# keras-team/keras-rs

Measured on AMD Instinct MI355X. Metric: embedding lookups/sec + DCN fwd+bwd step time, 26-table DLRM batch 65 536, higher is better.
Workload: dtype bf16; 1 GPU; C3 DLRM-small: 26 tables x 1000000 rows x 128 (bf16), global batch 65536, multi-hot ml_perf lengths (sum L = 214), uniform ids, DotInteraction(F=27) + 3 x FeatureCross(d=3456, projection=512), fused Adagrad on tables; global_batch=65536, parallelism=single GPU

## Files before the change

include/krs.h:

```cpp
#ifndef KRS_H_
#define KRS_H_

#include <stddef.h>
#include <stdint.h>

#ifdef __cplusplus
extern "C" {
#endif

#define KRS_VERSION 100

typedef enum krs_status {
  KRS_OK = 0,
  KRS_ERR_INVALID = -1,
  KRS_ERR_UNSUPPORTED = -2,
  KRS_ERR_LAUNCH = -3,
  KRS_ERR_WORKSPACE = -4
} krs_status;

typedef enum krs_dtype { KRS_F32 = 0, KRS_BF16 = 1, KRS_I8 = 2 } krs_dtype;
typedef enum krs_itype { KRS_I32 = 0, KRS_I64 = 1 } krs_itype;

typedef enum krs_combiner { KRS_SUM = 0, KRS_MEAN = 1, KRS_SQRTN = 2 } krs_combiner;

// ... 169 lines not shown
int krs_gemm_dense_bwd(const void* a, int64_t lda, const void* bt, int64_t ldb, void* g_out, int64_t ldg,
                       const void* y, void* dz, int64_t ld, float* dbias, int64_t m, int64_t n, int64_t k, int act,
                       int dtype, void* workspace, size_t workspace_bytes, void* stream);
enum { KRS_CROSS_BWD_NONE = 0, KRS_CROSS_BWD_TWO_CALL = 1, KRS_CROSS_BWD_PP64 = 2, KRS_CROSS_BWD_PP256 = 3 };
int krs_gemm_cross_bwd_last_route(int* epilogue);
int krs_gemm_cross_bwd_plan_route(const void* a, int64_t lda, const void* bt, int64_t ldb, const void* r, int64_t ldr,
                                  float beta, void* g_out, int64_t ldg, const void* x0, const void* u, void* dz, void* dx0,
                                  int64_t ld, int dx0_accumulate, const void* u_upper, int64_t m, int64_t n, int64_t k,
                                  int dtype, int* epilogue);

enum {
  KRS_GEMM_KERNEL_NONE = 0, KRS_GEMM_KERNEL_GENERIC = 1, KRS_GEMM_KERNEL_MFMA = 2, KRS_GEMM_KERNEL_GLDS = 3,
  KRS_GEMM_KERNEL_TN_GLDS = 4, KRS_GEMM_KERNEL_PP256 = 5, KRS_GEMM_KERNEL_PP256_KSTRIDED = 6, KRS_GEMM_KERNEL_PP64 = 7,
  KRS_GEMM_KERNEL_THIN = 8, KRS_GEMM_KERNEL_ROWDOT = 9, KRS_GEMM_KERNEL_SMALLK = 10
};
enum { KRS_GEMM_REDUCE_NONE = 0, KRS_GEMM_REDUCE_SCALAR = 1, KRS_GEMM_REDUCE_VEC4 = 2, KRS_GEMM_REDUCE_VEC8 = 3 };
typedef struct krs_gemm_route {
  int32_t kernel;
  int32_t splits;
  int32_t reduce;
  int32_t epilogue;
  int32_t ep_vec;
  int32_t thin_width;
  int32_t thin_is_a;
} krs_gemm_route;
int krs_gemm_last_route(krs_gemm_route* route);
int krs_gemm_plan_route(const void* a, int64_t lda, int a_is_km, const void* b, int64_t ldb, int b_is_nk, const void* c,
                        int64_t ldc, int64_t m, int64_t n, int64_t k, int in_dtype, int out_dtype,
                        const krs_gemm_epilogue* epilogue, size_t workspace_bytes, krs_gemm_route* route);

enum { KRS_GEMM_OPT_PIPELINE = 0 };
int krs_gemm_set_option(int key, int value);

enum { KRS_EMBED_OPT_PLAN = 2, KRS_EMBED_OPT_HOTROWS = 3, KRS_EMBED_OPT_RANK = 4, KRS_EMBED_OPT_APPLY_DEPTH = 5 };
int krs_embed_set_option(int key, int value);

size_t krs_colsum_workspace_bytes(int64_t m, int64_t n);
int krs_cross_epilogue_fwd(const void* u, const void* x0, const void* x, void* y,
                           int64_t m, int64_t n, int64_t ld, float diag_scale,
                           int dtype, void* stream);
int krs_cross_epilogue_bwd(const void* g, const void* u, const void* x0, const void* x,
                           void* du, void* dx0, int dx0_accumulate, void* dxd,
                           float* dbias,
                           int64_t m, int64_t n, int64_t ld, float diag_scale, int act,
                           int dtype, void* workspace, size_t workspace_bytes, void* stream);

int krs_cast_transpose(const void* src, int64_t rows, int64_t cols, int64_t ld_src, int src_dtype,
                       void* dst, int64_t ld_dst, void* dst_t, int64_t ld_dst_t, int dst_dtype,
                       void* stream);
int krs_cast_transpose_many(int count, const void* const* srcs, const int64_t* rows, const int64_t* cols,
                            int src_dtype, void* const* dsts, void* const* dst_ts, int dst_dtype, void* stream);

int krs_dense_act_bwd(const void* g, int64_t ld_g, const void* y, int64_t ld_y, void* dz, int64_t ld_dz,
                      float* dbias, int64_t m, int64_t n, int act, int dtype, void* workspace,
                      size_t workspace_bytes, void* stream);

int krs_dense_adagrad(float* const* params, const float* const* grads, float* const* accs,
                      const int64_t* sizes, int count, float lr, float eps, void* stream);

int krs_colsum(const void* a, int64_t lda, int64_t m, int64_t n, int dtype,
               float* out, void* workspace, size_t workspace_bytes, void* stream);

int krs_dot_interaction_fwd(const void* const* feats, const int64_t* ld, int n_feats,
                            int64_t batch, int dim, int dtype,
                            int self_interaction, int skip_gather,
                            void* out, int64_t out_ld, void* stream);
int krs_dot_interaction_bwd(const void* const* feats, const int64_t* ld, int n_feats,
// ... 150 lines not shown
```

keras_rs_amd/csrc/embed_bag_fwd.hip:

```cpp
#include <cstdlib>

#include "embed_fwd_plan.h"
#include "krs_common.h"

namespace krs {
namespace {

typedef uint32_t u32x4 __attribute__((ext_vector_type(4)));
typedef float f32x4 __attribute__((ext_vector_type(4)));
constexpr int NT = 2;

struct EmbedFwdParams {
  const krs_table* tables;
  const krs_feature* feats;
  int n_feats;
  const void* ids;
  int id64;
  const void* offsets;
  int off64;
  const float* weights;
  int batch;
  int dim;
  void* out;
  int64_t out_ld;
// ... 521 lines not shown
    if constexpr (sizeof(TT) == 2 && sizeof(OT) == 2 && LPR == 16) {
      if (rt.hot_rows == 128) {
        if (rt.stream) hipLaunchKernelGGL((embed_bag_fwd_vec<TT, OT, LPR, false, true, 128>), grid, block, 0, st, p);
        else hipLaunchKernelGGL((embed_bag_fwd_vec<TT, OT, LPR, false, false, 128>), grid, block, 0, st, p);
      } else {
        if (rt.stream) hipLaunchKernelGGL((embed_bag_fwd_vec<TT, OT, LPR, false, true, 64>), grid, block, 0, st, p);
        else hipLaunchKernelGGL((embed_bag_fwd_vec<TT, OT, LPR, false, false, 64>), grid, block, 0, st, p);
      }
      KRS_CHECK_LAUNCH("embed_bag_fwd_vec (hot rows in LDS)");
      return KRS_OK;
    } else {
      return fail(KRS_ERR_UNSUPPORTED, "embed_bag_fwd: hot rows are staged for bf16 rows of 256 bytes only");
    }
  }
#define KRS_K1_LAUNCH(W, S) hipLaunchKernelGGL((embed_bag_fwd_vec<TT, OT, LPR, W, S>), grid, block, 0, st, p)
  if (rt.has_w) { if (rt.stream) KRS_K1_LAUNCH(true, true); else KRS_K1_LAUNCH(true, false); }
  else { if (rt.stream) KRS_K1_LAUNCH(false, true); else KRS_K1_LAUNCH(false, false); }
#undef KRS_K1_LAUNCH
  KRS_CHECK_LAUNCH("embed_bag_fwd_vec");
  return KRS_OK;
}

template <typename TT, typename OT>
int launch_vec(const EmbedFwdParams& p, const krs_embed_fwd_route& rt, hipStream_t st) {
  if (rt.lpr == 8) return launch_lpr<TT, OT, 8>(p, rt, st);
  if (rt.lpr == 16) return launch_lpr<TT, OT, 16>(p, rt, st);
  if (rt.lpr == 32) return launch_lpr<TT, OT, 32>(p, rt, st);
  return launch_lpr<TT, OT, 64>(p, rt, st);
}

}
}

namespace krs { extern int g_plan_variant, g_rank_mode; }
namespace krs { int g_apply_depth = 4; }

extern "C" int krs_embed_set_option(int key, int value) {
  if (key == KRS_EMBED_OPT_PLAN) {
    KRS_REQUIRE(value == 0 || value == 1, "krs_embed_set_option: plan variant must be 0 or 1");
    krs::g_plan_variant = value;
    return KRS_OK;
  }
  if (key == KRS_EMBED_OPT_RANK) {
    KRS_REQUIRE(value >= 0 && value <= 2, "krs_embed_set_option: rank mode must be 0, 1 or 2");
    krs::g_rank_mode = value;
    return KRS_OK;
  }
  if (key == KRS_EMBED_OPT_HOTROWS) {
    KRS_REQUIRE(value == 0 || value == 64 || value == 128, "krs_embed_set_option: hot rows must be 0, 64 or 128");
    krs::g_hot_rows = value;
    return KRS_OK;
  }
  if (key == KRS_EMBED_OPT_APPLY_DEPTH) {
    KRS_REQUIRE(value == 0 || value == 4 || value == 8 || value == 16,
                "krs_embed_set_option: apply depth must be 0, 4, 8 or 16");
    krs::g_apply_depth = value;
    return KRS_OK;
  }
  return krs::fail(KRS_ERR_INVALID, "krs_embed_set_option: unknown key %d", key);
}

extern "C" int krs_embed_bag_fwd(const krs_table* tables, const krs_feature* feats, int n_feats,
                                 const void* ids, int id_type, const void* offsets, int off_type,
                                 const float* weights, int64_t nnz, int batch, int dim,
                                 int table_dtype, void* out, int out_dtype, int64_t out_ld,
                                 float* bag_scale, int* err_flag, void* stream) {
  using namespace krs;
  g_route = krs_embed_fwd_route{};
  KRS_REQUIRE(tables && feats && out, "embed_bag_fwd: null tables/feats/out");
  KRS_REQUIRE(ids || nnz == 0, "embed_bag_fwd: null ids");
  eplan::EmbedFwdPlan pl;
  if (int rc = embed_fwd_plan(n_feats, offsets, weights, nnz, batch, dim, table_dtype, out, out_dtype, out_ld, pl)) return rc;
  KRS_REQUIRE((id_type == KRS_I32 || id_type == KRS_I64) && (off_type == KRS_I32 || off_type == KRS_I64),
              "embed_bag_fwd: bad index type");
  const krs_embed_fwd_route& rt = pl.route;
  if (rt.kernel == KRS_EMBED_FWD_NONE) return KRS_OK;
  hipStream_t st = reinterpret_cast<hipStream_t>(stream);

// ... 36 lines not shown
```

keras_rs_amd/csrc/embed_bag_plan.hip:

```cpp
#include <algorithm>

#include "krs_bag_plan.h"

namespace krs {
int g_plan_variant = 0;
int g_rank_mode = 0;
namespace {

namespace rs {
constexpr int kHistThreads = 256, kHistItems = kTile / kHistThreads;
constexpr int kThreads = 512, kWaves = kThreads / 64, kItems = kTile / kThreads;
constexpr int kGenFeats = 256;

struct Gen {
  const krs_table* tables;
  const krs_feature* feats;
  int n_feats;
  const void* ids;
  int id64;
  int batch;
  int* err_flag;
};

struct alignas(16) GenLds {
  uint32_t base[kGenFeats + 1];
  uint32_t hot[kGenFeats];
  uint32_t row_base[kGenFeats];
  uint32_t vocab[kGenFeats];
};
__device__ __forceinline__ void load_gen(const Gen& gen, int64_t nnz, GenLds& g, int n_threads) {
  for (int i = threadIdx.x; i <= gen.n_feats; i += n_threads) {
    if (i < gen.n_feats) {
      const krs_feature ft = gen.feats[i];
      const krs_table tb = gen.tables[ft.table];
      g.base[i] = (uint32_t)ft.ids_base;
      g.hot[i] = (uint32_t)ft.hot;
      g.row_base[i] = (uint32_t)tb.row_base;
      g.vocab[i] = (uint32_t)tb.vocab;
    } else {
      g.base[i] = (uint32_t)nnz;
    }
  }
}
__device__ __forceinline__ int gen_feature(const GenLds& g, int n_feats, uint32_t q) {
  int lo = 0, hi = n_feats;
  while (hi - lo > 1) {
    const int mid = (lo + hi) >> 1;
    if (g.base[mid] <= q) lo = mid; else hi = mid;
  }
  return lo;
}
__device__ __forceinline__ uint64_t gen_value(const Gen& gen, const GenLds& g, int f, uint32_t q) {
  const uint32_t bag = (uint32_t)f * (uint32_t)gen.batch + (q - g.base[f]) / g.hot[f];
  return ((uint64_t)bag << 32) | (uint64_t)q;
}
__device__ __forceinline__ bool generate(const Gen& gen, const GenLds& g, uint32_t q, uint32_t& key, uint64_t& val) {
  const int f = gen_feature(g, gen.n_feats, q);
  const int64_t id = ld_index(gen.ids, gen.id64, q);
  const bool valid = id >= 0 && id < (int64_t)g.vocab[f];
  key = valid ? g.row_base[f] + (uint32_t)id : kInvalidKey;
  val = gen_value(gen, g, f, q);
  return valid;
}

__device__ __forceinline__ int digit_of(uint32_t key, int shift, int bins) { return (int)((key >> shift) & (bins - 1)); }

__device__ __forceinline__ uint32_t tile_of_block(uint32_t b, uint32_t tiles) { return (b & 7) * ((tiles + 7) / 8) + (b >> 3); }
inline unsigned tile_grid(unsigned tiles) { return (tiles + 7) / 8 * 8; }

__device__ __forceinline__ void hist_zero(int (&h)[kMaxBins], int bins) {
  for (int i = threadIdx.x; i < bins; i += kHistThreads) h[i] = 0;
}
__device__ __forceinline__ void hist_add(int (&h)[kMaxBins], uint32_t key, int shift, int bins) {
  atomicAdd(&h[digit_of(key, shift, bins)], 1);
}
__device__ __forceinline__ void hist_finish(const int (&h)[kMaxBins], int bins, int32_t* col, int64_t stride, bool bad,
                                            int* err_flag) {
  if (bad && err_flag) atomicOr(err_flag, KRS_FLAG_ID_OUT_OF_RANGE);
  __syncthreads();
  for (int i = threadIdx.x; i < bins; i += kHistThreads) col[(int64_t)i * stride] = h[i];
}

template <typename V>
struct alignas(16) TileLds {
  uint16_t cnt[kWaves][kMaxBins];
  uint16_t tile_excl[kMaxBins];
  int gbase[kMaxBins];
  uint32_t skey[kTile];
  V sval[kTile];
  int wtot[kWaves];
};
template <typename V>
__device__ __forceinline__ void zero_counts(TileLds<V>& s) {
  for (int i = threadIdx.x; i < kWaves * kMaxBins; i += kThreads) (&s.cnt[0][0])[i] = 0;
}
// ... 110 lines not shown
    }
  }
  __syncthreads();
}
template <typename V>
__device__ __forceinline__ void stage_tile(TileLds<V>& s, const uint32_t (&key)[kItems], const V (&val)[kItems],
                                           const int (&rank)[kItems], int64_t first, int64_t end, int shift, int bins) {
  const int wave = threadIdx.x >> 6;
#pragma unroll
  for (int it = 0; it < kItems; ++it) {
    if (first + it * 64 < end) {
      const int lp = s.cnt[wave][digit_of(key[it], shift, bins)] + rank[it];
      s.skey[lp] = key[it];
      s.sval[lp] = val[it];
    }
  }
  __syncthreads();
}
template <typename V>
__device__ __forceinline__ int out_slot(const TileLds<V>& s, int i, int d) {
  return s.gbase[d] + (i - (int)s.tile_excl[d]);
}

struct Pass {
  const uint32_t* keys_in;
  const uint64_t* vals_in;
  uint32_t* keys_out;
  uint64_t* vals_out;
  int32_t* counts;
  int64_t nnz;
  int n_tiles;
  int shift, bits;
  int rank;
  Gen gen;
};

template <bool GEN>
__global__ __launch_bounds__(kHistThreads) void hist_kernel(const Pass p) {
  __shared__ int h[kMaxBins];
  __shared__ GenLds g;
  const uint32_t tile = tile_of_block(blockIdx.x, p.n_tiles);
  if (tile >= (uint32_t)p.n_tiles) return;
  const int bins = 1 << p.bits;
  hist_zero(h, bins);
  if constexpr (GEN) load_gen(p.gen, p.nnz, g, kHistThreads);
  __syncthreads();
  const int64_t base = (int64_t)tile * kTile;
  bool bad = false;
  for (int it = 0; it < kHistItems; ++it) {
    const int64_t q = base + it * kHistThreads + threadIdx.x;
    if (q < p.nnz) {
      uint32_t key;
      if constexpr (GEN) {
        uint64_t v;
        bad |= !generate(p.gen, g, (uint32_t)q, key, v);
      } else {
        key = p.keys_in[q];
      }
      hist_add(h, key, p.shift, bins);
    }
  }
  hist_finish(h, bins, p.counts + tile, p.n_tiles, bad, p.gen.err_flag);
}

template <bool GEN>
__global__ __launch_bounds__(kThreads) void scatter_kernel(const Pass p) {
  __shared__ TileLds<uint64_t> s;
  __shared__ GenLds g;
  const uint32_t tile = tile_of_block(blockIdx.x, p.n_tiles);
  if (tile >= (uint32_t)p.n_tiles) return;
  const int bins = 1 << p.bits;
  zero_counts(s);
  if constexpr (GEN) load_gen(p.gen, p.nnz, g, kThreads);
  __syncthreads();
  const int lane = threadIdx.x & 63, wave = threadIdx.x >> 6;
  const int64_t tile0 = (int64_t)tile * kTile;
  const int64_t first = tile0 + (int64_t)wave * (kTile / kWaves) + lane;
  uint32_t key[kItems];
  uint64_t val[kItems];
  int rank[kItems];
#pragma unroll
  for (int it = 0; it < kItems; ++it) {
    const int64_t q = first + it * 64;
    const bool live = q < p.nnz;
    key[it] = kInvalidKey;
    val[it] = 0;
    if (live) {
      if constexpr (GEN) {
        generate(p.gen, g, (uint32_t)q, key[it], val[it]);
      } else {
        key[it] = p.keys_in[q];
        val[it] = p.vals_in[q];
      }
    }
  }
  rank_keys(key, first, p.nnz, p.shift, p.bits, p.rank, s.cnt[wave], lane, rank);
  digit_bases(s, bins, p.counts + tile, p.n_tiles);
  stage_tile(s, key, val, rank, first, p.nnz, p.shift, bins);
  const int n_here = (int)min<int64_t>(kTile, p.nnz - tile0);
#pragma unroll
  for (int it = 0; it < kItems; ++it) {
    const int i = it * kThreads + threadIdx.x;
    if (i < n_here) {
      const uint32_t k = s.skey[i];
      const int pos = out_slot(s, i, digit_of(k, p.shift, bins));
      p.keys_out[pos] = k;
      p.vals_out[pos] = s.sval[i];
    }
  }
}

struct Seg {
  int n;
  uint32_t lookup_start[kMaxProb + 1];
  uint32_t tile_start[kMaxProb + 1];
  uint32_t row_base[kMaxProb];
};
struct SegPass {
  const uint32_t* keys_in;
  const uint32_t* pos_in;
  uint32_t* keys_out;
  uint32_t* pos_out;
  uint64_t* vals_out;
  int32_t* counts;
  int64_t nnz;
  int shift, bits, key_bits;
  int rank;
  Gen gen;
  Seg seg;
};
struct SegTile {
  int pr;
  int64_t t0, end;
  int32_t* col;
  uint32_t stride;
};
__device__ __forceinline__ SegTile seg_tile(const SegPass& p, uint32_t tile) {
  const Seg& sg = p.seg;
  int lo = 0, hi = sg.n;
  while (hi - lo > 1) {
    const int mid = (lo + hi) >> 1;
    if (sg.tile_start[mid] <= tile) lo = mid; else hi = mid;
  }
  SegTile t;
  t.pr = lo;
  const uint32_t tl = tile - sg.tile_start[lo];
  t.stride = sg.tile_start[lo + 1] - sg.tile_start[lo];
  t.t0 = (int64_t)sg.lookup_start[lo] + (int64_t)tl * kTile;
  t.end = min<int64_t>(t.t0 + kTile, sg.lookup_start[lo + 1]);
  t.col = p.counts + ((int64_t)1 << p.bits) * sg.tile_start[lo] + tl;
  return t;
}
template <int ITEMS, int STRIDE>
__device__ __forceinline__ bool seg_first_keys(const SegPass& p, const GenLds& g, const SegTile& t, int64_t first,
                                               uint32_t (&key)[ITEMS], uint32_t (&pos)[ITEMS]) {
  int64_t idv[ITEMS];
#pragma unroll
  for (int it = 0; it < ITEMS; ++it) idv[it] = ld_index(p.gen.ids, p.gen.id64, min<int64_t>(first + it * STRIDE, t.end - 1));
  const int f_lo = gen_feature(g, p.gen.n_feats, (uint32_t)t.t0), f_hi = gen_feature(g, p.gen.n_feats, (uint32_t)(t.end - 1));
  bool bad = false;
#pragma unroll
  for (int it = 0; it < ITEMS; ++it) {
    const int64_t q = min<int64_t>(first + it * STRIDE, t.end - 1);
    const int f = f_lo == f_hi ? f_lo : gen_feature(g, p.gen.n_feats, (uint32_t)q);
    const bool valid = idv[it] >= 0 && idv[it] < (int64_t)g.vocab[f];
    key[it] = valid ? (uint32_t)idv[it] : (1u << p.key_bits) - 1u;
    pos[it] = (uint32_t)q;
    bad = bad || (!valid && first + it * STRIDE < t.end);
  }
  return bad;
}

template <bool FIRST>
__global__ __launch_bounds__(kHistThreads) void hist_seg_kernel(const SegPass p) {
  __shared__ int h[kMaxBins];
  __shared__ GenLds g;
  const uint32_t tile = tile_of_block(blockIdx.x, p.seg.tile_start[p.seg.n]);
  if (tile >= p.seg.tile_start[p.seg.n]) return;
  const int bins = 1 << p.bits;
  hist_zero(h, bins);
  if constexpr (FIRST) load_gen(p.gen, p.nnz, g, kHistThreads);
  __syncthreads();
  const SegTile t = seg_tile(p, tile);
  const int64_t first = t.t0 + threadIdx.x;
  bool bad = false;
  uint32_t key[kHistItems];
  if constexpr (FIRST) {
    uint32_t pos[kHistItems];
    bad = seg_first_keys<kHistItems, kHistThreads>(p, g, t, first, key, pos);
  } else {
#pragma unroll
    for (int it = 0; it < kHistItems; ++it) key[it] = p.keys_in[min<int64_t>(first + it * kHistThreads, t.end - 1)];
  }
#pragma unroll
  for (int it = 0; it < kHistItems; ++it)
    if (first + it * kHistThreads < t.end) hist_add(h, key[it], p.shift, bins);
  hist_finish(h, bins, t.col, t.stride, bad, p.gen.err_flag);
}

template <bool FIRST, bool LAST>
__global__ __launch_bounds__(kThreads) void scatter_seg_kernel(const SegPass p) {
  __shared__ TileLds<uint32_t> s;
  __shared__ GenLds g;
  const uint32_t tile = tile_of_block(blockIdx.x, p.seg.tile_start[p.seg.n]);
  if (tile >= p.seg.tile_start[p.seg.n]) return;
  const int bins = 1 << p.bits;
  zero_counts(s);
  if constexpr (FIRST || LAST) load_gen(p.gen, p.nnz, g, kThreads);
  __syncthreads();
  const int lane = threadIdx.x & 63, wave = threadIdx.x >> 6;
  const SegTile t = seg_tile(p, tile);
  const int64_t first = t.t0 + (int64_t)wave * (kTile / kWaves) + lane;
  uint32_t key[kItems], pos[kItems];
  int rank[kItems];
  if constexpr (FIRST) {
    seg_first_keys<kItems, 64>(p, g, t, first, key, pos);
  } else {
#pragma unroll
    for (int it = 0; it < kItems; ++it) {
      const int64_t q = min<int64_t>(first + it * 64, t.end - 1);
      key[it] = p.keys_in[q];
      pos[it] = p.pos_in[q];
    }
  }
#pragma unroll
  for (int it = 0; it < kItems; ++it) {
    const bool live = first + it * 64 < t.end;
    if (!live) { key[it] = 0xffffffffu; pos[it] = 0; }
  }
  rank_keys(key, first, t.end, p.shift, p.bits, p.rank, s.cnt[wave], lane, rank);
  digit_bases(s, bins, t.col, t.stride);
  stage_tile(s, key, pos, rank, first, t.end, p.shift, bins);
  const int n_here = (int)(t.end - t.t0);
  const uint32_t sentinel = (1u << p.key_bits) - 1u, rb = p.seg.row_base[t.pr];
  int pf_lo = 0, pf_hi = 1;
  if constexpr (LAST) {
    pf_lo = gen_feature(g, p.gen.n_feats, p.seg.lookup_start[t.pr]);
    pf_hi = gen_feature(g, p.gen.n_feats, p.seg.lookup_start[t.pr + 1] - 1);
  }
#pragma unroll
  for (int it = 0; it < kItems; ++it) {
    const int i = it * kThreads + threadIdx.x;
    if (i < n_here) {
      const uint32_t k = s.skey[i], q = s.sval[i];
      const int o = out_slot(s, i, digit_of(k, p.shift, bins));
      if constexpr (LAST) {
        const int f = pf_lo == pf_hi ? pf_lo : gen_feature(g, p.gen.n_feats, q);
        p.keys_out[o] = k == sentinel ? kInvalidKey : rb + k;
        p.vals_out[o] = gen_value(p.gen, g, f, q);
      } else {
        p.keys_out[o] = k;
        p.pos_out[o] = q;
      }
    }
  }
}

inline unsigned key_bits(int64_t n) {
  unsigned bits = 1;
  while (bits < 32 && (1ULL << bits) <= (uint64_t)n) ++bits;
  return bits;
}
struct Schedule {
  int passes;
  int bits[4], shift[4];
};
inline Schedule pass_schedule(unsigned bits) {
  Schedule s;
  s.passes = (int)((bits + kMaxBits - 1) / kMaxBits);
  unsigned done = 0;
  for (int ps = 0; ps < s.passes; ++ps) {
    s.bits[ps] = (int)((bits - done + (s.passes - ps) - 1) / (s.passes - ps));
    s.shift[ps] = (int)done;
    done += (unsigned)s.bits[ps];
  }
  return s;
}
inline Gen make_gen(const krs_table* tables, const krs_feature* feats, int n_feats, const void* ids, int id_type,
                    int batch, int* err_flag) {
  Gen g;
  g.tables = tables; g.feats = feats; g.n_feats = n_feats; g.ids = ids;
  g.id64 = id_type == KRS_I64; g.batch = batch; g.err_flag = err_flag;
  return g;
}
}

struct KeyParams {
  const krs_table* tables;
  const krs_feature* feats;
  int n_feats;
  const void* ids;
  int id64;
  const void* offsets;
  int off64;
  int batch;
  uint32_t* keys;
  uint64_t* vals;
  int* err_flag;
};

__global__ __launch_bounds__(256) void bag_keys_kernel(const KeyParams p) {
  const int64_t bag = (int64_t)blockIdx.x * 16 + (threadIdx.x >> 4);
  const int sub = threadIdx.x & 15;
  if (bag >= (int64_t)p.n_feats * p.batch) return;
  const int f = (int)(bag / p.batch);
  const int b = (int)(bag - (int64_t)f * p.batch);
  const krs_feature ft = p.feats[f];
  const krs_table tb = p.tables[ft.table];
  int64_t s, e;
  if (p.offsets) {
    s = ld_index(p.offsets, p.off64, bag);
    e = ld_index(p.offsets, p.off64, bag + 1);
  } else {
    s = ft.ids_base + (int64_t)b * ft.hot;
    e = s + ft.hot;
// ... 57 lines not shown
#pragma unroll
  for (int o = 1; o < 64; o <<= 1) {
    const int y = __shfl_up(x, o, 64);
    if (lane >= o) x += y;
  }
  if (lane == 63) wsum[wave] = x;
  __syncthreads();
  uint32_t off = (uint32_t)block_off[blockIdx.x] + (uint32_t)(x - c);
  for (int w = 0; w < wave; ++w) off += (uint32_t)wsum[w];
  uint32_t m = mask;
  while (m) {
    const int k = __ffs(m) - 1;
    m &= m - 1;
    seg_start[off++] = (uint32_t)(t0 + k);
  }
  if (t0 < nnz && t0 + kSegItems >= nnz) *n_seg = off;
}
__global__ void long_list_kernel(const uint32_t* seg_start, const uint32_t* n_seg, int64_t nnz, uint32_t* counters,
                                 LongItem* items, MultiSeg* multi) {
  const int64_t u = (int64_t)blockIdx.x * blockDim.x + threadIdx.x;
  const uint32_t ns = *n_seg;
  if (u >= ns) return;
  const int64_t e = u + 1 < ns ? (int64_t)seg_start[u + 1] : nnz;
  const int64_t len = e - (int64_t)seg_start[u];
  if (len <= kLongSeg) return;
  const uint32_t nch = (uint32_t)((len + kChunk - 1) / kChunk);
  const uint32_t base = atomicAdd(counters, nch);
  uint32_t pb = 0xffffffffu;
  if (nch > 1) {
    pb = atomicAdd(counters + 1, nch);
    multi[atomicAdd(counters + 2, 1u)] = MultiSeg{(uint32_t)u, pb, nch};
  }
  for (uint32_t c = 0; c < nch; ++c) items[base + c] = LongItem{(uint32_t)u, c, nch > 1 ? pb + c : 0xffffffffu};
}

bool plan_sort_by_table(const PlanLayout& l, const rs::Temp& tmp, const rs::Gen& gen, const krs_table* tables_host,
                        int n_tables, const krs_feature* feats_host, int64_t nnz, hipStream_t st) {
  if (!tables_host || !feats_host || gen.n_feats > rs::kGenFeats || n_tables <= 0) return false;
  rs::SegPass sp;
  rs::Seg& sg = sp.seg;
  sg.n = 0;
  int64_t pos = 0, max_vocab = 0;
  int prev_table = -1;
  for (int f = 0; f < gen.n_feats; ++f) {
    const krs_feature& ft = feats_host[f];
    if (ft.hot < 1 || ft.ids_base != pos || ft.table < prev_table || ft.table >= n_tables) return false;
    if (ft.table != prev_table) {
      if (sg.n == rs::kMaxProb) return false;
      const krs_table& tb = tables_host[ft.table];
      if (prev_table >= 0 && tb.row_base < tables_host[prev_table].row_base + tables_host[prev_table].vocab) return false;
      sg.lookup_start[sg.n] = (uint32_t)pos;
      sg.row_base[sg.n] = (uint32_t)tb.row_base;
      max_vocab = std::max<int64_t>(max_vocab, tb.vocab);
      ++sg.n;
      prev_table = ft.table;
    }
    pos += (int64_t)gen.batch * ft.hot;
  }
  if (pos != nnz || sg.n == 0) return false;
  sg.lookup_start[sg.n] = (uint32_t)nnz;
  uint32_t tiles = 0;
  for (int i = 0; i < sg.n; ++i) {
    sg.tile_start[i] = tiles;
    tiles += (uint32_t)ceil_div((int64_t)sg.lookup_start[i + 1] - sg.lookup_start[i], rs::kTile);
  }
  sg.tile_start[sg.n] = tiles;
  if (tiles == 0) return false;
  const unsigned bits = rs::key_bits(max_vocab);
  if (bits > 31) return false;
  const rs::Schedule sch = rs::pass_schedule(bits);
  sp.counts = tmp.counts; sp.nnz = nnz; sp.key_bits = (int)bits; sp.rank = g_rank_mode;
  sp.gen = gen;
  uint32_t* k0 = l.keys_in; uint32_t* q0 = reinterpret_cast<uint32_t*>(l.vals_in);
  uint32_t* k1 = l.keys_sorted; uint32_t* q1 = reinterpret_cast<uint32_t*>(l.vals_sorted);
  for (int ps = 0; ps < sch.passes; ++ps) {
    const bool first = ps == 0, last = ps == sch.passes - 1;
    sp.bits = sch.bits[ps];
    sp.shift = sch.shift[ps];
    const bool out_is_i0 = ((sch.passes - 2 - ps) % 2) == 0;
    const bool in_is_i0 = ((sch.passes - 1 - ps) % 2) == 0;
    sp.keys_in = first ? nullptr : (in_is_i0 ? k0 : k1);
    sp.pos_in = first ? nullptr : (in_is_i0 ? q0 : q1);
    sp.keys_out = last ? l.keys_sorted : (out_is_i0 ? k0 : k1);
    sp.pos_out = last ? nullptr : (out_is_i0 ? q0 : q1);
    sp.vals_out = last ? l.vals_sorted : nullptr;
    if (first) hipLaunchKernelGGL(rs::hist_seg_kernel<true>, dim3(rs::tile_grid(tiles)), dim3(rs::kHistThreads), 0, st, sp);
    else hipLaunchKernelGGL(rs::hist_seg_kernel<false>, dim3(rs::tile_grid(tiles)), dim3(rs::kHistThreads), 0, st, sp);
    scan::exclusive(tmp.counts, tmp.counts, (int64_t)(1 << sp.bits) * tiles, tmp.sums, nullptr, st);
    if (first && last) hipLaunchKernelGGL((rs::scatter_seg_kernel<true, true>), dim3(rs::tile_grid(tiles)), dim3(rs::kThreads), 0, st, sp);
    else if (first) hipLaunchKernelGGL((rs::scatter_seg_kernel<true, false>), dim3(rs::tile_grid(tiles)), dim3(rs::kThreads), 0, st, sp);
    else if (last) hipLaunchKernelGGL((rs::scatter_seg_kernel<false, true>), dim3(rs::tile_grid(tiles)), dim3(rs::kThreads), 0, st, sp);
    else hipLaunchKernelGGL((rs::scatter_seg_kernel<false, false>), dim3(rs::tile_grid(tiles)), dim3(rs::kThreads), 0, st, sp);
  }
  return true;
}

int plan_sort_global(const PlanLayout& l, const rs::Temp& tmp, const rs::Gen& gen, const void* offsets, int off_type,
                     int64_t nnz, int64_t total_rows, hipStream_t st) {
  const rs::Schedule sch = rs::pass_schedule(rs::key_bits(total_rows));
  const bool gen_first = offsets == nullptr && gen.n_feats <= rs::kGenFeats;
  bool to_sorted = (sch.passes % 2) == 1;
  if (!gen_first) {
    KeyParams kp;
    kp.tables = gen.tables; kp.feats = gen.feats; kp.n_feats = gen.n_feats; kp.ids = gen.ids; kp.id64 = gen.id64;
    kp.offsets = offsets; kp.off64 = off_type == KRS_I64; kp.batch = gen.batch; kp.err_flag = gen.err_flag;
    kp.keys = to_sorted ? l.keys_in : l.keys_sorted;
    kp.vals = to_sorted ? l.vals_in : l.vals_sorted;
    const int64_t n_bags = (int64_t)gen.n_feats * gen.batch;
    KRS_HIP(hipMemsetAsync(kp.keys, 0xff, (size_t)nnz * sizeof(uint32_t), st));
    hipLaunchKernelGGL(bag_keys_kernel, dim3((unsigned)ceil_div(n_bags, 16)), dim3(256), 0, st, kp);
    KRS_CHECK_LAUNCH("bag_keys_kernel");
  }
  rs::Pass p;
  p.nnz = nnz;
  p.n_tiles = (int)ceil_div(nnz, rs::kTile);
  p.counts = tmp.counts;
  p.rank = g_rank_mode;
  p.gen = gen;
  for (int ps = 0; ps < sch.passes; ++ps) {
    p.bits = sch.bits[ps];
    p.shift = sch.shift[ps];
    const bool generating = gen_first && ps == 0;
    p.keys_in = generating ? nullptr : (to_sorted ? l.keys_in : l.keys_sorted);
    p.vals_in = generating ? nullptr : (to_sorted ? l.vals_in : l.vals_sorted);
    p.keys_out = to_sorted ? l.keys_sorted : l.keys_in;
    p.vals_out = to_sorted ? l.vals_sorted : l.vals_in;
    if (generating) hipLaunchKernelGGL(rs::hist_kernel<true>, dim3(rs::tile_grid((unsigned)p.n_tiles)), dim3(rs::kHistThreads), 0, st, p);
    else hipLaunchKernelGGL(rs::hist_kernel<false>, dim3(rs::tile_grid((unsigned)p.n_tiles)), dim3(rs::kHistThreads), 0, st, p);
    scan::exclusive(tmp.counts, tmp.counts, (int64_t)(1 << p.bits) * p.n_tiles, tmp.sums, nullptr, st);
    if (generating) hipLaunchKernelGGL(rs::scatter_kernel<true>, dim3(rs::tile_grid((unsigned)p.n_tiles)), dim3(rs::kThreads), 0, st, p);
    else hipLaunchKernelGGL(rs::scatter_kernel<false>, dim3(rs::tile_grid((unsigned)p.n_tiles)), dim3(rs::kThreads), 0, st, p);
    to_sorted = !to_sorted;
  }
  return KRS_OK;
}

int plan_impl(const krs_table* tables, const krs_table* tables_host, int n_tables, const krs_feature* feats,
              const krs_feature* feats_host, int n_feats, const void* ids, int id_type, const void* offsets,
              int off_type, int batch, int64_t nnz, int64_t total_rows, void* workspace, size_t workspace_bytes,
              int* err_flag, void* stream) {
  KRS_REQUIRE(tables && feats && (ids || nnz == 0), "embed_bag_bwd_plan: null argument");
  KRS_REQUIRE(n_feats > 0 && batch > 0 && nnz >= 0, "embed_bag_bwd_plan: bad sizes");
  KRS_REQUIRE(total_rows > 0 && total_rows < 0xffffffffLL, "embed_bag_bwd_plan: total_rows must fit 32-bit keys");
  KRS_REQUIRE(nnz < 0x7fffffffLL && (int64_t)n_feats * batch < 0xffffffffLL,
              "embed_bag_bwd_plan: nnz must stay below 2^31 and the bag count below 2^32");
  if (nnz == 0) return KRS_OK;
  KRS_REQUIRE(workspace, "embed_bag_bwd_plan: null workspace");
  const PlanLayout l = plan_layout(workspace, nnz, true);
  if (workspace_bytes < l.total_bytes)
    return fail(KRS_ERR_WORKSPACE, "embed_bag_bwd_plan: workspace %zu < %zu bytes", workspace_bytes, l.total_bytes);
  hipStream_t st = reinterpret_cast<hipStream_t>(stream);
  const rs::Temp tmp = rs::carve_temp(l.temp, nnz);
  const rs::Gen gen = rs::make_gen(tables, feats, n_feats, ids, id_type, batch, err_flag);
  const bool by_table = offsets == nullptr && g_plan_variant == 0 &&
                        plan_sort_by_table(l, tmp, gen, tables_host, n_tables, feats_host, nnz, st);
  if (!by_table)
    if (int rc = plan_sort_global(l, tmp, gen, offsets, off_type, nnz, total_rows, st)) return rc;
  KRS_CHECK_LAUNCH("embed_bag_bwd_plan: radix sort");
  const unsigned nb = (unsigned)ceil_div(nnz, 256);
  const unsigned nsb = (unsigned)ceil_div(nnz, kSegTile);
  hipLaunchKernelGGL(seg_count_kernel, dim3(nsb), dim3(256), 0, st, l.keys_sorted, nnz, tmp.sums2);
  hipLaunchKernelGGL(scan::block_kernel, dim3(1), dim3(1024), 0, st, tmp.sums2, (int64_t)nsb, (int64_t*)nullptr);
  hipLaunchKernelGGL(seg_emit_kernel, dim3(nsb), dim3(256), 0, st, l.keys_sorted, nnz, tmp.sums2, l.seg_start, l.n_seg);
  KRS_CHECK_LAUNCH("seg_emit_kernel");
  KRS_HIP(hipMemsetAsync(l.n_long, 0, 3 * sizeof(uint32_t), st));
  KRS_HIP(hipMemsetAsync(l.sort_mode, by_table ? 1 : 0, sizeof(uint32_t), st));
  hipLaunchKernelGGL(long_list_kernel, dim3(nb), dim3(256), 0, st, l.seg_start, l.n_seg, nnz, l.n_long, l.long_list,
                     l.multi_list);
  KRS_CHECK_LAUNCH("long_list_kernel");
  return KRS_OK;
}

}
}

using namespace krs;

extern "C" size_t krs_embed_bag_bwd_workspace_bytes(int64_t nnz) {
  if (nnz < 0) return 0;
  return plan_layout(nullptr, nnz, true).total_bytes;
}

extern "C" int krs_embed_bag_bwd_plan(const krs_table* tables, const krs_feature* feats, int n_feats,
                                      const void* ids, int id_type, const void* offsets, int off_type,
                                      int batch, int64_t nnz, int64_t total_rows, void* workspace,
                                      size_t workspace_bytes, int* err_flag, void* stream) {
  return plan_impl(tables, nullptr, 0, feats, nullptr, n_feats, ids, id_type, offsets, off_type, batch, nnz, total_rows,
                   workspace, workspace_bytes, err_flag, stream);
}

extern "C" int krs_embed_bag_bwd_plan_tables(const krs_table* tables, const krs_table* tables_host, int n_tables,
                                             const krs_feature* feats, const krs_feature* feats_host, int n_feats,
                                             const void* ids, int id_type, int batch, int64_t nnz, int64_t total_rows,
// ... 6 lines not shown
```

Before: 1.501 billion lookups/s.

## Specialize single-feature plan tiles and fuse segment count/scan/emit kernels

Radix-sort generation passes now detect tiles that lie within one feature and load ids in a vectorized way, with a precomputed reciprocal in place of integer division for bag indices. This skips the per-element binary search and division. The segment planning stage fuses count, scan and the long-list memsets into one last-block-ticket kernel, and emits long segments inline. That cuts several launches and memsets, and a reference switch keeps the old path available. The cost is more complex cross-block synchronization through a ticket counter and more LDS and argument state.

```diff
diff --git a/include/krs.h b/include/krs.h
--- a/include/krs.h
+++ b/include/krs.h
@@ -225,7 +225,8 @@
 enum { KRS_GEMM_OPT_PIPELINE = 0 };
 int krs_gemm_set_option(int key, int value);
 
-enum { KRS_EMBED_OPT_PLAN = 2, KRS_EMBED_OPT_HOTROWS = 3, KRS_EMBED_OPT_RANK = 4, KRS_EMBED_OPT_APPLY_DEPTH = 5 };
+enum { KRS_EMBED_OPT_PLAN = 2, KRS_EMBED_OPT_HOTROWS = 3, KRS_EMBED_OPT_RANK = 4, KRS_EMBED_OPT_APPLY_DEPTH = 5,
+       KRS_EMBED_OPT_PLAN_REF = 6 };
 int krs_embed_set_option(int key, int value);
 
 size_t krs_colsum_workspace_bytes(int64_t m, int64_t n);
diff --git a/keras_rs_amd/csrc/bag_recip.h b/keras_rs_amd/csrc/bag_recip.h
--- /dev/null
+++ b/keras_rs_amd/csrc/bag_recip.h
@@ -0,0 +1,33 @@
+#ifndef KRS_BAG_RECIP_H_
+#define KRS_BAG_RECIP_H_
+
+#include <stdint.h>
+
+#if defined(__HIPCC__)
+#define KRS_RECIP_FN __host__ __device__ inline
+#else
+#define KRS_RECIP_FN inline
+#endif
+
+namespace krs {
+namespace recip {
+
+struct Recip {
+  uint32_t mul, shift;
+};
+
+KRS_RECIP_FN Recip make(uint32_t d) {
+  if (d == 0) d = 1;
+  uint32_t l = 0;
+  while (l < 31 && (1u << l) < d) ++l;
+  Recip r;
+  r.mul = (uint32_t)((((uint64_t)1 << (31 + l)) + d - 1) / d);
+  r.shift = l;
+  return r;
+}
+
+KRS_RECIP_FN uint32_t div(uint32_t x, Recip r) { return (uint32_t)(((uint64_t)(x << 1) * r.mul) >> 32) >> r.shift; }
+
+}
+}
+#endif
diff --git a/keras_rs_amd/csrc/embed_bag_fwd.hip b/keras_rs_amd/csrc/embed_bag_fwd.hip
--- a/keras_rs_amd/csrc/embed_bag_fwd.hip
+++ b/keras_rs_amd/csrc/embed_bag_fwd.hip
@@ -577,7 +577,7 @@
 }
 }
 
-namespace krs { extern int g_plan_variant, g_rank_mode; }
+namespace krs { extern int g_plan_variant, g_rank_mode, g_plan_ref; }
 namespace krs { int g_apply_depth = 4; }
 
 extern "C" int krs_embed_set_option(int key, int value) {
@@ -589,6 +589,11 @@
   if (key == KRS_EMBED_OPT_RANK) {
     KRS_REQUIRE(value >= 0 && value <= 2, "krs_embed_set_option: rank mode must be 0, 1 or 2");
     krs::g_rank_mode = value;
+    return KRS_OK;
+  }
+  if (key == KRS_EMBED_OPT_PLAN_REF) {
+    KRS_REQUIRE(value == 0 || value == 1, "krs_embed_set_option: plan reference switch must be 0 or 1");
+    krs::g_plan_ref = value;
     return KRS_OK;
   }
   if (key == KRS_EMBED_OPT_HOTROWS) {
diff --git a/keras_rs_amd/csrc/embed_bag_plan.hip b/keras_rs_amd/csrc/embed_bag_plan.hip
--- a/keras_rs_amd/csrc/embed_bag_plan.hip
+++ b/keras_rs_amd/csrc/embed_bag_plan.hip
@@ -1,10 +1,12 @@
 #include <algorithm>
 
+#include "bag_recip.h"
 #include "krs_bag_plan.h"
 
 namespace krs {
 int g_plan_variant = 0;
 int g_rank_mode = 0;
+int g_plan_ref = 0;
 namespace {
 
 namespace rs {
@@ -20,6 +22,7 @@
   int id64;
   int batch;
   int* err_flag;
+  int ref;
 };
 
 struct alignas(16) GenLds {
@@ -27,7 +30,9 @@
   uint32_t hot[kGenFeats];
   uint32_t row_base[kGenFeats];
   uint32_t vocab[kGenFeats];
+  recip::Recip rhot[kGenFeats];
 };
+template <bool RECIP>
 __device__ __forceinline__ void load_gen(const Gen& gen, int64_t nnz, GenLds& g, int n_threads) {
   for (int i = threadIdx.x; i <= gen.n_feats; i += n_threads) {
     if (i < gen.n_feats) {
@@ -37,6 +42,8 @@
       g.hot[i] = (uint32_t)ft.hot;
       g.row_base[i] = (uint32_t)tb.row_base;
       g.vocab[i] = (uint32_t)tb.vocab;
+      if constexpr (RECIP)
+        if (!gen.ref) g.rhot[i] = recip::make((uint32_t)ft.hot);
     } else {
       g.base[i] = (uint32_t)nnz;
     }
@@ -61,6 +68,52 @@
   key = valid ? g.row_base[f] + (uint32_t)id : kInvalidKey;
   val = gen_value(gen, g, f, q);
   return valid;
+}
+
+struct GenFeat {
+  uint32_t base, vocab, row_base, bag0;
+  recip::Recip rhot;
+};
+template <bool RECIP>
+__device__ __forceinline__ GenFeat gen_feat(const Gen& gen, const GenLds& g, int f) {
+  GenFeat c;
+  c.base = g.base[f]; c.vocab = g.vocab[f]; c.row_base = g.row_base[f];
+  c.bag0 = (uint32_t)f * (uint32_t)gen.batch;
+  if constexpr (RECIP) c.rhot = g.rhot[f]; else c.rhot = recip::Recip{0u, 0u};
+  return c;
+}
+__device__ __forceinline__ uint64_t feat_value(const GenFeat& c, uint32_t q) {
+  return ((uint64_t)(c.bag0 + recip::div(q - c.base, c.rhot)) << 32) | (uint64_t)q;
+}
+template <typename I, int ITEMS, int STRIDE>
+__device__ __forceinline__ bool feat_ids(const void* ids, uint32_t vocab, uint32_t first, uint32_t end, uint32_t invalid,
+                                         uint32_t (&id)[ITEMS], uint32_t (&pos)[ITEMS]) {
+  const I* src = reinterpret_cast<const I*>(ids);
+  I raw[ITEMS];
+#pragma unroll
+  for (int it = 0; it < ITEMS; ++it) {
+    pos[it] = min(first + (uint32_t)(it * STRIDE), end - 1u);
+    raw[it] = src[pos[it]];
+  }
+  bool bad = false;
+#pragma unroll
+  for (int it = 0; it < ITEMS; ++it) {
+    const bool valid = raw[it] >= 0 && (uint64_t)raw[it] < (uint64_t)vocab;
+    id[it] = valid ? (uint32_t)raw[it] : invalid;
+    bad = bad || (!valid && first + (uint32_t)(it * STRIDE) < end);
+  }
+  return bad;
+}
+template <int ITEMS, int STRIDE>
+__device__ __forceinline__ bool feat_ids(const Gen& gen, uint32_t vocab, uint32_t first, uint32_t end, uint32_t invalid,
+                                         uint32_t (&id)[ITEMS], uint32_t (&pos)[ITEMS]) {
+  return gen.id64 ? feat_ids<int64_t, ITEMS, STRIDE>(gen.ids, vocab, first, end, invalid, id, pos)
+                  : feat_ids<int32_t, ITEMS, STRIDE>(gen.ids, vocab, first, end, invalid, id, pos);
+}
+__device__ __forceinline__ int tile_feature(const Gen& gen, const GenLds& g, uint32_t t0, uint32_t end) {
+  if (gen.ref) return -1;
+  const int f_lo = gen_feature(g, gen.n_feats, t0);
+  return f_lo == gen_feature(g, gen.n_feats, end - 1u) ? f_lo : -1;
 }
 
 __device__ __forceinline__ int digit_of(uint32_t key, int shift, int bins) { return (int)((key >> shift) & (bins - 1)); }
@@ -237,6 +290,7 @@
   int n_tiles;
   int shift, bits;
   int rank;
+  uint32_t* ticket;
   Gen gen;
 };
 
@@ -247,22 +301,35 @@
   const uint32_t tile = tile_of_block(blockIdx.x, p.n_tiles);
   if (tile >= (uint32_t)p.n_tiles) return;
   const int bins = 1 << p.bits;
+  if (blockIdx.x == 0 && threadIdx.x == 0) *p.ticket = 0u;
   hist_zero(h, bins);
-  if constexpr (GEN) load_gen(p.gen, p.nnz, g, kHistThreads);
+  if constexpr (GEN) load_gen<false>(p.gen, p.nnz, g, kHistThreads);
   __syncthreads();
   const int64_t base = (int64_t)tile * kTile;
   bool bad = false;
-  for (int it = 0; it < kHistItems; ++it) {
-    const int64_t q = base + it * kHistThreads + threadIdx.x;
-    if (q < p.nnz) {
-      uint32_t key;
-      if constexpr (GEN) {
-        uint64_t v;
-        bad |= !generate(p.gen, g, (uint32_t)q, key, v);
-      } else {
-        key = p.keys_in[q];
+  int f_tile = -1;
+  if constexpr (GEN) f_tile = tile_feature(p.gen, g, (uint32_t)base, (uint32_t)min<int64_t>(base + kTile, p.nnz));
+  if (f_tile >= 0) {
+    const uint32_t first = (uint32_t)base + threadIdx.x, end = (uint32_t)min<int64_t>(base + kTile, p.nnz);
+    const GenFeat c = gen_feat<false>(p.gen, g, f_tile);
+    uint32_t id[kHistItems], pos[kHistItems];
+    bad = feat_ids<kHistItems, kHistThreads>(p.gen, c.vocab, first, end, kInvalidKey - c.row_base, id, pos);
+#pragma unroll
+    for (int it = 0; it < kHistItems; ++it)
+      if (first + (uint32_t)(it * kHistThreads) < end) hist_add(h, c.row_base + id[it], p.shift, bins);
+  } else {
+    for (int it = 0; it < kHistItems; ++it) {
+      const int64_t q = base + it * kHistThreads + threadIdx.x;
+      if (q < p.nnz) {
+        uint32_t key;
+        if constexpr (GEN) {
+          uint64_t v;
+          bad |= !generate(p.gen, g, (uint32_t)q, key, v);
+        } else {
+          key = p.keys_in[q];
+        }
+        hist_add(h, key, p.shift, bins);
       }
-      hist_add(h, key, p.shift, bins);
     }
   }
   hist_finish(h, bins, p.counts + tile, p.n_tiles, bad, p.gen.err_flag);
@@ -276,7 +343,7 @@
   if (tile >= (uint32_t)p.n_tiles) return;
   const int bins = 1 << p.bits;
   zero_counts(s);
-  if constexpr (GEN) load_gen(p.gen, p.nnz, g, kThreads);
+  if constexpr (GEN) load_gen<true>(p.gen, p.nnz, g, kThreads);
   __syncthreads();
   const int lane = threadIdx.x & 63, wave = threadIdx.x >> 6;
   const int64_t tile0 = (int64_t)tile * kTile;
@@ -284,18 +351,33 @@
   uint32_t key[kItems];
   uint64_t val[kItems];
   int rank[kItems];
-#pragma unroll
-  for (int it = 0; it < kItems; ++it) {
-    const int64_t q = first + it * 64;
-    const bool live = q < p.nnz;
-    key[it] = kInvalidKey;
-    val[it] = 0;
-    if (live) {
-      if constexpr (GEN) {
-        generate(p.gen, g, (uint32_t)q, key[it], val[it]);
-      } else {
-        key[it] = p.keys_in[q];
-        val[it] = p.vals_in[q];
+  int f_tile = -1;
+  if constexpr (GEN) f_tile = tile_feature(p.gen, g, (uint32_t)tile0, (uint32_t)min<int64_t>(tile0 + kTile, p.nnz));
+  if (f_tile >= 0) {
+    const uint32_t end = (uint32_t)min<int64_t>(tile0 + kTile, p.nnz);
+    const GenFeat c = gen_feat<true>(p.gen, g, f_tile);
+    uint32_t id[kItems], pos[kItems];
+    feat_ids<kItems, 64>(p.gen, c.vocab, (uint32_t)first, end, kInvalidKey - c.row_base, id, pos);
+#pragma unroll
+    for (int it = 0; it < kItems; ++it) {
+      const bool live = (uint32_t)first + (uint32_t)(it * 64) < end;
+      key[it] = live ? c.row_base + id[it] : kInvalidKey;
+      val[it] = live ? feat_value(c, pos[it]) : 0;
+    }
+  } else {
+#pragma unroll
+    for (int it = 0; it < kItems; ++it) {
+      const int64_t q = first + it * 64;
+      const bool live = q < p.nnz;
+      key[it] = kInvalidKey;
+      val[it] = 0;
+      if (live) {
+        if constexpr (GEN) {
+          generate(p.gen, g, (uint32_t)q, key[it], val[it]);
+        } else {
+          key[it] = p.keys_in[q];
+          val[it] = p.vals_in[q];
+        }
       }
     }
   }
@@ -320,7 +402,11 @@
   uint32_t lookup_start[kMaxProb + 1];
   uint32_t tile_start[kMaxProb + 1];
   uint32_t row_base[kMaxProb];
+  uint32_t vocab[kMaxProb];
+  recip::Recip rhot[kMaxProb];
+  uint16_t one_feat[kMaxProb];
 };
+constexpr uint16_t kSeveralFeats = 0xffffu;
 struct SegPass {
   const uint32_t* keys_in;
   const uint32_t* pos_in;
@@ -331,9 +417,11 @@
   int64_t nnz;
   int shift, bits, key_bits;
   int rank;
+  uint32_t* ticket;
   Gen gen;
   Seg seg;
 };
+static_assert(sizeof(SegPass) <= 4096, "SegPass travels as a kernel argument");
 struct SegTile {
   int pr;
   int64_t t0, end;
@@ -383,8 +471,10 @@
   const uint32_t tile = tile_of_block(blockIdx.x, p.seg.tile_start[p.seg.n]);
   if (tile >= p.seg.tile_start[p.seg.n]) return;
   const int bins = 1 << p.bits;
+  if (blockIdx.x == 0 && threadIdx.x == 0) *p.ticket = 0u;
   hist_zero(h, bins);
-  if constexpr (FIRST) load_gen(p.gen, p.nnz, g, kHistThreads);
+  if constexpr (FIRST)
+    if (p.gen.ref) load_gen<false>(p.gen, p.nnz, g, kHistThreads);
   __syncthreads();
   const SegTile t = seg_tile(p, tile);
   const int64_t first = t.t0 + threadIdx.x;
@@ -392,7 +482,11 @@
   uint32_t key[kHistItems];
   if constexpr (FIRST) {
     uint32_t pos[kHistItems];
-    bad = seg_first_keys<kHistItems, kHistThreads>(p, g, t, first, key, pos);
+    if (!p.gen.ref)
+      bad = feat_ids<kHistItems, kHistThreads>(p.gen, p.seg.vocab[t.pr], (uint32_t)first, (uint32_t)t.end, (1u << p.key_bits) - 1u,
+                                               key, pos);
+    else
+      bad = seg_first_keys<kHistItems, kHistThreads>(p, g, t, first, key, pos);
   } else {
 #pragma unroll
     for (int it = 0; it < kHistItems; ++it) key[it] = p.keys_in[min<int64_t>(first + it * kHistThreads, t.end - 1)];
@@ -411,15 +505,22 @@
   if (tile >= p.seg.tile_start[p.seg.n]) return;
   const int bins = 1 << p.bits;
   zero_counts(s);
-  if constexpr (FIRST || LAST) load_gen(p.gen, p.nnz, g, kThreads);
+  const SegTile t = seg_tile(p, tile);
+  bool lds_gen = false;
+  if constexpr (FIRST || LAST) {
+    lds_gen = p.gen.ref || (LAST && p.seg.one_feat[t.pr] == kSeveralFeats);
+    if (lds_gen) load_gen<false>(p.gen, p.nnz, g, kThreads);
+  }
   __syncthreads();
   const int lane = threadIdx.x & 63, wave = threadIdx.x >> 6;
-  const SegTile t = seg_tile(p, tile);
   const int64_t first = t.t0 + (int64_t)wave * (kTile / kWaves) + lane;
   uint32_t key[kItems], pos[kItems];
   int rank[kItems];
   if constexpr (FIRST) {
-    seg_first_keys<kItems, 64>(p, g, t, first, key, pos);
+    if (!p.gen.ref)
+      feat_ids<kItems, 64>(p.gen, p.seg.vocab[t.pr], (uint32_t)first, (uint32_t)t.end, (1u << p.key_bits) - 1u, key, pos);
+    else
+      seg_first_keys<kItems, 64>(p, g, t, first, key, pos);
   } else {
 #pragma unroll
     for (int it = 0; it < kItems; ++it) {
@@ -439,9 +540,17 @@
   const int n_here = (int)(t.end - t.t0);
   const uint32_t sentinel = (1u << p.key_bits) - 1u, rb = p.seg.row_base[t.pr];
   int pf_lo = 0, pf_hi = 1;
+  GenFeat cf = {};
+  const bool one_feat = LAST && !lds_gen;
   if constexpr (LAST) {
-    pf_lo = gen_feature(g, p.gen.n_feats, p.seg.lookup_start[t.pr]);
-    pf_hi = gen_feature(g, p.gen.n_feats, p.seg.lookup_start[t.pr + 1] - 1);
+    if (one_feat) {
+      cf.base = p.seg.lookup_start[t.pr];
+      cf.bag0 = (uint32_t)p.seg.one_feat[t.pr] * (uint32_t)p.gen.batch;
+      cf.rhot = p.seg.rhot[t.pr];
+    } else {
+      pf_lo = gen_feature(g, p.gen.n_feats, p.seg.lookup_start[t.pr]);
+      pf_hi = gen_feature(g, p.gen.n_feats, p.seg.lookup_start[t.pr + 1] - 1);
+    }
   }
 #pragma unroll
   for (int it = 0; it < kItems; ++it) {
@@ -450,9 +559,13 @@
       const uint32_t k = s.skey[i], q = s.sval[i];
       const int o = out_slot(s, i, digit_of(k, p.shift, bins));
       if constexpr (LAST) {
-        const int f = pf_lo == pf_hi ? pf_lo : gen_feature(g, p.gen.n_feats, q);
         p.keys_out[o] = k == sentinel ? kInvalidKey : rb + k;
-        p.vals_out[o] = gen_value(p.gen, g, f, q);
+        if (one_feat) {
+          p.vals_out[o] = feat_value(cf, q);
+        } else {
+          const int f = pf_lo == pf_hi ? pf_lo : gen_feature(g, p.gen.n_feats, q);
+          p.vals_out[o] = gen_value(p.gen, g, f, q);
+        }
       } else {
         p.keys_out[o] = k;
         p.pos_out[o] = q;
@@ -486,6 +599,7 @@
   Gen g;
   g.tables = tables; g.feats = feats; g.n_feats = n_feats; g.ids = ids;
   g.id64 = id_type == KRS_I64; g.batch = batch; g.err_flag = err_flag;
+  g.ref = g_plan_ref;
   return g;
 }
 }
@@ -609,6 +723,157 @@
     multi[atomicAdd(counters + 2, 1u)] = MultiSeg{(uint32_t)u, pb, nch};
   }
   for (uint32_t c = 0; c < nch; ++c) items[base + c] = LongItem{(uint32_t)u, c, nch > 1 ? pb + c : 0xffffffffu};
+}
+
+constexpr uint32_t kNoHead = 0xffffffffu;
+inline uint32_t* tail_ticket(const rs::Temp& tmp, int64_t nnz) {
+  return reinterpret_cast<uint32_t*>(tmp.sums2) + ceil_div(nnz > 0 ? nnz : 1, kSegTile) + 1;
+}
+constexpr int kCountTiles = 8;
+__global__ __launch_bounds__(1024) void seg_count_scan_kernel(const uint32_t* keys, int64_t nnz, int32_t* block_heads,
+                                                              uint32_t nsb, uint32_t* ticket, uint32_t* n_long,
+                                                              uint32_t* sort_mode, uint32_t mode) {
+  __shared__ int total[kCountTiles];
+  __shared__ int wsum[16];
+  __shared__ int carry;
+  __shared__ uint32_t drawn;
+  if (threadIdx.x < kCountTiles) total[threadIdx.x] = 0;
+  __syncthreads();
+  const int lane = threadIdx.x & 63, wave = threadIdx.x >> 6;
+  const int quarter = threadIdx.x >> 8, tq = threadIdx.x & 255;
+  int c[kCountTiles / 4];
+#pragma unroll
+  for (int r = 0; r < kCountTiles / 4; ++r)
+    c[r] = __popc(seg_head_mask(keys, nnz, ((int64_t)blockIdx.x * kCountTiles + r * 4 + quarter) * kSegTile + tq * kSegItems));
+#pragma unroll
+  for (int r = 0; r < kCountTiles / 4; ++r) {
+    for (int o = 32; o; o >>= 1) c[r] += __shfl_down(c[r], o, 64);
+    if (lane == 0) atomicAdd(&total[r * 4 + quarter], c[r]);
+  }
+  __syncthreads();
+  if (wave == 0) {
+    const uint32_t b = blockIdx.x * kCountTiles + threadIdx.x;
+    if (blockIdx.x == 0 && threadIdx.x == 0) {
+      n_long[0] = 0u; n_long[1] = 0u; n_long[2] = 0u;
+      *sort_mode = mode;
+    }
+    if (threadIdx.x < kCountTiles && b < nsb)
+      __hip_atomic_store(block_heads + b, total[threadIdx.x], __ATOMIC_RELAXED, __HIP_MEMORY_SCOPE_AGENT);
+    asm volatile("s_waitcnt vmcnt(0)" ::: "memory");
+    if (threadIdx.x == 0) {
+      drawn = __hip_atomic_fetch_add(ticket, 1u, __ATOMIC_RELAXED, __HIP_MEMORY_SCOPE_AGENT);
+      carry = 0;
+    }
+  }
+  __syncthreads();
+  if (drawn != gridDim.x - 1) return;
+  for (uint32_t base = 0; base < nsb; base += 4096) {
+    int v[4];
+#pragma unroll
+    for (int k = 0; k < 4; ++k) {
+      const uint32_t i = base + k * 1024 + threadIdx.x;
+      v[k] = i < nsb ? __hip_atomic_load(block_heads + i, __ATOMIC_RELAXED, __HIP_MEMORY_SCOPE_AGENT) : 0;
+    }
+#pragma unroll
+    for (int k = 0; k < 4; ++k) {
+      const uint32_t i = base + k * 1024 + threadIdx.x;
+      int x = v[k];
+#pragma unroll
+      for (int o = 1; o < 64; o <<= 1) {
+        const int y = __shfl_up(x, o, 64);
+        if (lane >= o) x += y;
+      }
+      if (lane == 63) wsum[wave] = x;
+      __syncthreads();
+      int off = carry + x - v[k];
+      for (int w = 0; w < wave; ++w) off += wsum[w];
+      if (i < nsb) block_heads[i] = off;
+      __syncthreads();
+      if (threadIdx.x == 1023) carry = off + v[k];
+      __syncthreads();
+    }
+  }
+  if (threadIdx.x == 0) block_heads[nsb] = carry;
+}
+__device__ __forceinline__ void emit_long(uint32_t u, uint32_t len, uint32_t* counters, LongItem* items, MultiSeg* multi) {
+  const uint32_t nch = (len + kChunk - 1) / kChunk;
+  const uint32_t base = atomicAdd(counters, nch);
+  uint32_t pb = 0xffffffffu;
+  if (nch > 1) {
+    pb = atomicAdd(counters + 1, nch);
+    multi[atomicAdd(counters + 2, 1u)] = MultiSeg{u, pb, nch};
+  }
+  for (uint32_t c = 0; c < nch; ++c) items[base + c] = LongItem{u, c, nch > 1 ? pb + c : 0xffffffffu};
+}
+__global__ __launch_bounds__(256) void seg_emit_long_kernel(const uint32_t* keys, int64_t nnz, const int32_t* block_off,
+                                                            uint32_t* seg_start, uint32_t* n_seg, uint32_t* counters,
+                                                            LongItem* items, MultiSeg* multi) {
+  __shared__ int wsum[4];
+  __shared__ uint32_t wmin[4];
+  __shared__ uint32_t s_next, s_blk;
+  const int64_t t0 = (int64_t)blockIdx.x * kSegTile + threadIdx.x * kSegItems;
+  const uint32_t mask = seg_head_mask(keys, nnz, t0);
+  if (threadIdx.x == 255) {
+    const int64_t e = (int64_t)(blockIdx.x + 1) * kSegTile;
+    uint32_t nx = (uint32_t)nnz;
+    if (e < nnz) {
+      const uint32_t m = seg_head_mask(keys, nnz, e);
+      nx = m ? (uint32_t)e + (uint32_t)(__ffs(m) - 1) : (e + kSegItems >= nnz ? (uint32_t)nnz : kNoHead);
+    }
+    s_next = nx;
+    s_blk = kNoHead;
+  }
+  const int c = __popc(mask), lane = threadIdx.x & 63, wave = threadIdx.x >> 6;
+  int x = c;
+  uint32_t sm = mask ? (uint32_t)t0 + (uint32_t)(__ffs(mask) - 1) : kNoHead;
+#pragma unroll
+  for (int o = 1; o < 64; o <<= 1) {
+    const int y = __shfl_up(x, o, 64);
+    if (lane >= o) x += y;
+    const uint32_t z = __shfl_down(sm, o, 64);
+    if (lane + o < 64) sm = min(sm, z);
+  }
+  uint32_t nxt = __shfl_down(sm, 1, 64);
+  if (lane == 63) { nxt = kNoHead; wsum[wave] = x; }
+  if (lane == 0) wmin[wave] = sm;
+  __syncthreads();
+  uint32_t past = s_next;
+  const bool has_head = min(min(wmin[0], wmin[1]), min(wmin[2], wmin[3])) != kNoHead;
+  __syncthreads();
+  if (past == kNoHead && has_head) {
+    const uint32_t nsb = gridDim.x;
+    for (uint32_t base = blockIdx.x + 1; base < nsb; base += 256) {
+      const uint32_t b2 = base + threadIdx.x;
+      if (b2 < nsb && block_off[b2 + 1] != block_off[b2]) atomicMin(&s_blk, b2);
+      __syncthreads();
+      const uint32_t found = s_blk;
+      __syncthreads();
+      if (found != kNoHead) break;
+    }
+    const uint32_t fb = s_blk;
+    past = (uint32_t)nnz;
+    if (fb != kNoHead) {
+      const int64_t t2 = (int64_t)fb * kSegTile + threadIdx.x * kSegItems;
+      const uint32_t m2 = seg_head_mask(keys, nnz, t2);
+      if (m2) atomicMin(&s_next, (uint32_t)t2 + (uint32_t)(__ffs(m2) - 1));
+      __syncthreads();
+      past = s_next;
+    }
+  }
+  for (int w = wave + 1; w < 4; ++w) nxt = min(nxt, wmin[w]);
+  nxt = min(nxt, past);
+  uint32_t off = (uint32_t)block_off[blockIdx.x] + (uint32_t)(x - c);
+  for (int w = 0; w < wave; ++w) off += (uint32_t)wsum[w];
+  uint32_t m = mask;
+  while (m) {
+    const uint32_t h = (uint32_t)t0 + (uint32_t)(__ffs(m) - 1);
+    m &= m - 1;
+    const uint32_t len = (m ? (uint32_t)t0 + (uint32_t)(__ffs(m) - 1) : nxt) - h;
+    seg_start[off] = h;
+    if (len > (uint32_t)kLongSeg) emit_long(off, len, counters, items, multi);
+    ++off;
+  }
+  if (t0 < nnz && t0 + kSegItems >= nnz) *n_seg = off;
 }
 
 bool plan_sort_by_table(const PlanLayout& l, const rs::Temp& tmp, const rs::Gen& gen, const krs_table* tables_host,
@@ -628,9 +893,14 @@
       if (prev_table >= 0 && tb.row_base < tables_host[prev_table].row_base + tables_host[prev_table].vocab) return false;
       sg.lookup_start[sg.n] = (uint32_t)pos;
       sg.row_base[sg.n] = (uint32_t)tb.row_base;
+      sg.vocab[sg.n] = (uint32_t)tb.vocab;
+      sg.rhot[sg.n] = recip::make((uint32_t)ft.hot);
+      sg.one_feat[sg.n] = (uint16_t)f;
       max_vocab = std::max<int64_t>(max_vocab, tb.vocab);
       ++sg.n;
       prev_table = ft.table;
+    } else {
+      sg.one_feat[sg.n - 1] = rs::kSeveralFeats;
     }
     pos += (int64_t)gen.batch * ft.hot;
   }
@@ -647,6 +917,7 @@
   if (bits > 31) return false;
   const rs::Schedule sch = rs::pass_schedule(bits);
   sp.counts = tmp.counts; sp.nnz = nnz; sp.key_bits = (int)bits; sp.rank = g_rank_mode;
+  sp.ticket = tail_ticket(tmp, nnz);
   sp.gen = gen;
   uint32_t* k0 = l.keys_in; uint32_t* q0 = reinterpret_cast<uint32_t*>(l.vals_in);
   uint32_t* k1 = l.keys_sorted; uint32_t* q1 = reinterpret_cast<uint32_t*>(l.vals_sorted);
@@ -693,6 +964,7 @@
   p.n_tiles = (int)ceil_div(nnz, rs::kTile);
   p.counts = tmp.counts;
   p.rank = g_rank_mode;
+  p.ticket = tail_ticket(tmp, nnz);
   p.gen = gen;
   for (int ps = 0; ps < sch.passes; ++ps) {
     p.bits = sch.bits[ps];
@@ -736,6 +1008,15 @@
   KRS_CHECK_LAUNCH("embed_bag_bwd_plan: radix sort");
   const unsigned nb = (unsigned)ceil_div(nnz, 256);
   const unsigned nsb = (unsigned)ceil_div(nnz, kSegTile);
+  if (!g_plan_ref) {
+    hipLaunchKernelGGL(seg_count_scan_kernel, dim3((unsigned)ceil_div((int64_t)nsb, kCountTiles)), dim3(1024), 0, st, l.keys_sorted, nnz,
+                       tmp.sums2, nsb, tail_ticket(tmp, nnz),
+                       l.n_long, l.sort_mode, by_table ? 0x01010101u : 0u);
+    hipLaunchKernelGGL(seg_emit_long_kernel, dim3(nsb), dim3(256), 0, st, l.keys_sorted, nnz, tmp.sums2, l.seg_start, l.n_seg,
+                       l.n_long, l.long_list, l.multi_list);
+    KRS_CHECK_LAUNCH("seg_emit_long_kernel");
+    return KRS_OK;
+  }
   hipLaunchKernelGGL(seg_count_kernel, dim3(nsb), dim3(256), 0, st, l.keys_sorted, nnz, tmp.sums2);
   hipLaunchKernelGGL(scan::block_kernel, dim3(1), dim3(1024), 0, st, tmp.sums2, (int64_t)nsb, (int64_t*)nullptr);
   hipLaunchKernelGGL(seg_emit_kernel, dim3(nsb), dim3(256), 0, st, l.keys_sorted, nnz, tmp.sums2, l.seg_start, l.n_seg);
```

Result: no change. 1.509 billion lookups/s (median of 6 runs) (+0.5%).
